# snakers4/silero-vad

Measured on AMD Instinct MI355X. Metric: audio-chunks/sec (32 ms @ 16 kHz), higher is better.
Workload: dtype f32; 1 GPU; configs[1]: synthetic 16 kHz PCM resident in HBM, 512-sample chunks, 4096 streams/GPU x 256 chunks/stream per step, zero initial state; streams_per_gpu=4096

## Files before the change

silero_vad_amd/csrc/device_api.hpp:

```cpp
#pragma once
#include <hip/hip_runtime.h>

#include <cstdint>

#include "../../include/silero_vad_hip.h"

namespace vad {

struct RefNet {
    const float *basis;
    const float *ew[4], *eb[4];
    const float *w_ih, *w_hh, *b_ih, *b_hh, *w_out, *b_out;
};

__device__ __forceinline__ float load_pcm(const float *p) { return *p; }
__device__ __forceinline__ float load_pcm(const int16_t *p) { return (float)(*p) * (1.0f / 32768.0f); }

template <typename PcmT>
hipError_t launch_ref_forward(const RefNet &w, int sr, int B, long L, const PcmT *pcm, long ld,
                              float *ctx, float *state, float *probs, long ldp, hipStream_t s);

template <typename PcmT>
hipError_t launch_decimate(const PcmT *src, long lds, PcmT *dst, long ldd, int B, long Ld, int k, hipStream_t s);

struct FrontArgs {
    const float *wfront;
    const float *tables;
    const void *pcm;
    const void *tail;
    long ld, L, T;
    long t0, nt;
    const float *ctx_in;
    float *ctx_out;
    float *gx;
    int B;
    int dec;
    long long *trace;
    const RefNet *exact_net;
    int *exact_list;
    const float *gx_silent;
};
hipError_t launch_exact_silent(int sr, const RefNet *net_dev, float *out, hipStream_t s);
template <typename PcmT>
hipError_t launch_exact_fix(int sr, const FrontArgs &a, hipStream_t s);
template <typename PcmT>
hipError_t launch_front(int sr, const FrontArgs &a, hipStream_t s);
template <typename PcmT>
hipError_t launch_front_f43(int sr, const FrontArgs &a, hipStream_t s);
template <typename PcmT>
hipError_t launch_front_lat(int sr, const FrontArgs &a, hipStream_t s);
struct CellArgs {
    const float *whh_lat;
    float *state;
    float *probs;
    long ldp;
    const uint8_t *present;
};
template <typename PcmT>
hipError_t launch_step_lat(int sr, const FrontArgs &a, const CellArgs &c, hipStream_t s);
template <typename PcmT>
hipError_t launch_step_one(int sr, const FrontArgs &a, const CellArgs &c, hipStream_t s);
template <typename PcmT>
hipError_t launch_front_one(int sr, const FrontArgs &a, hipStream_t s);
template <typename PcmT>
hipError_t launch_front_wino(int sr, const FrontArgs &a, hipStream_t s);

struct RecArgs {
    const float *whh;
    const float *tables;
    const float *gx;
    float *state;
    float *probs;
    long ldp, t0, nt;
    int B;
    const uint8_t *present;
};
hipError_t launch_rec(int sr, const RecArgs &a, hipStream_t s);
hipError_t launch_carry_absent(const uint8_t *present, const float *ctx_in, float *ctx_out, int C, float *probs, long ldp, int B,
                               hipStream_t s);
hipError_t launch_expand_rows(const uint8_t *present, const int32_t *pos, const uint8_t *src, void *dst, long row_bytes, int B, hipStream_t s);
hipError_t launch_assemble_packets(const int32_t *table, long n_rows, const int16_t *pkt, int16_t *carry, int16_t *batch, int N, hipStream_t s);
constexpr int kCodecShift = 16;
hipError_t launch_assemble_coded_packets(const int32_t *table, long n_rows, const uint8_t *pkt, int16_t *carry, int16_t *batch, int N,
                                         hipStream_t s);
hipError_t launch_assemble_burst(const int32_t *table, long n_rows, const uint8_t *pkt, int16_t *carry, int16_t *batch, int16_t *more,
                                 int max_chunks, int streams, int N, hipStream_t s);
hipError_t launch_burst_flags(const uint8_t *k_of_stream, uint8_t *flags, long ld, int steps, int streams, hipStream_t s);

__host__ __device__ inline int16_t ulaw_to_s16(uint8_t code) {
    const unsigned u = ~code & 0xffu;
    const int t = (int)((((u & 0x0fu) << 3) + 0x84u) << ((u & 0x70u) >> 4));
    return (int16_t)((u & 0x80u) ? 0x84 - t : t - 0x84);
}
__host__ __device__ inline int16_t alaw_to_s16(uint8_t code) {
    const unsigned a = code ^ 0x55u;
    const unsigned seg = (a & 0x70u) >> 4;
    const int m = (int)((a & 0x0fu) << 4);
    const int t = seg == 0 ? m + 8 : (m + 0x108) << (seg - 1);
    return (int16_t)((a & 0x80u) ? t : -t);
}
__host__ __device__ inline int16_t g711_to_s16(int codec, uint8_t code) {
// ... 26 lines not shown
```

silero_vad_amd/csrc/engine.hip:

```cpp
#include <hip/hip_runtime.h>

#include <chrono>

#include <sched.h>

#include <algorithm>
#include <atomic>
#include <cctype>
#include <cstdio>
#include <cstdlib>
#include <cstring>
#include <map>
#include <memory>
#include <mutex>
#include <new>
#include <string>
#include <vector>

#include "../../include/silero_vad_hip.h"
#include "device_api.hpp"
#include "host_threads.hpp"
#include "layout.hpp"
#include "weights.hpp"

#ifndef VAD_AB
#define VAD_AB 0
#endif

struct vad_images {
    int device = -1;
    uint8_t *d_blob = nullptr;
    vad::RefNet ref[2] = {};
    vad::RefNet *d_ref = nullptr;
    float *d_gx_silent = nullptr;
    float *d_front4[2] = {}, *d_whh[2] = {}, *d_whh_lat[2] = {}, *d_whh_rows[2] = {}, *d_tables[2] = {};
    uint16_t *d_whh_b9[2] = {}, *d_front_b9[2] = {};
#if VAD_AB
    float *d_front[2] = {}, *d_front_wino[2] = {};
#endif
    ~vad_images() {
        if (device < 0) return;
        (void)hipSetDevice(device);
        for (int ni = 0; ni < 2; ++ni) {
            if (d_front4[ni]) (void)hipFree(d_front4[ni]);
            if (d_whh[ni]) (void)hipFree(d_whh[ni]);
            if (d_whh_b9[ni]) (void)hipFree(d_whh_b9[ni]);
            if (d_whh_rows[ni]) (void)hipFree(d_whh_rows[ni]);
            if (d_front_b9[ni]) (void)hipFree(d_front_b9[ni]);
            if (d_whh_lat[ni]) (void)hipFree(d_whh_lat[ni]);
            if (d_tables[ni]) (void)hipFree(d_tables[ni]);
#if VAD_AB
            if (d_front[ni]) (void)hipFree(d_front[ni]);
            if (d_front_wino[ni]) (void)hipFree(d_front_wino[ni]);
#endif
        }
        if (d_blob) (void)hipFree(d_blob);
        if (d_ref) (void)hipFree(d_ref);
        if (d_gx_silent) (void)hipFree(d_gx_silent);
    }
};

struct vad_engine {
    std::shared_ptr<vad::Weights> weights;
    std::shared_ptr<vad_images> img;
    bool host_only = false;
    int device = -1;
    std::string err;
    bool impl_reference = false;
    int enc0 = 2;
    bool fuse_step = true;
    int rec_form = 0;
    bool front_b9 = false;
    bool rec_b9 = false;
    bool profile = false;
    bool fused_decimation = true;
    bool exact_all_silent = true;
    bool exact_transitions = true;
    int one_max = 256;
    long lat_tiles = 768;
    long long *trace = nullptr;

    float *d_gx = nullptr;
    size_t gx_floats = 0;
    float *d_ctx_new = nullptr;
    size_t ctx_floats = 0;
    int *d_exact = nullptr;
    size_t exact_ints = 0;
    void *d_tail = nullptr;
    size_t tail_bytes = 0;
    void *d_realign = nullptr;
    size_t realign_bytes = 0;
    void *d_decim = nullptr;
    size_t decim_bytes = 0;
    unsigned long scratch_gen = 0;
    long slab_steps = 0;
    size_t gx_cap = 6ull << 30;

    static constexpr int kTabSlots = 8;
    vad::RowDesc *h_tab[kTabSlots] = {};
    long tab_cap[kTabSlots] = {};
    hipEvent_t tab_ev[kTabSlots] = {};
    bool tab_busy[kTabSlots] = {};
    int tab_next = 0;

    static constexpr int kDmaStreams = 4;
    hipStream_t dma_stream[kDmaStreams] = {};
    hipEvent_t dma_fork = nullptr, dma_join[kDmaStreams] = {};

    const void *map_host[2] = {nullptr, nullptr};
    void *map_dev[2] = {nullptr, nullptr};
    unsigned long map_gen = 0;

    std::vector<hipEvent_t> ev_pool;
    size_t ev_used = 0;
    long prof_calls = 0;
};

namespace {

int fail(vad_engine *e, int code, const std::string &msg) {
    if (e) e->err = msg;
    return code;
}
// ... 147 lines not shown
        ra.tables = e->img->d_tables[ni];
        ra.gx = e->d_gx;
        ra.state = state;
        ra.probs = probs;
        ra.ldp = ldp; ra.t0 = t0; ra.nt = nt; ra.B = B;
        ra.present = present;
        hipEvent_t *ev = nullptr;
        if (prof) {
            while (e->ev_pool.size() < e->ev_used + 3) {
                hipEvent_t x;
                HIP_TRY(e, hipEventCreate(&x));
                e->ev_pool.push_back(x);
            }
            ev = &e->ev_pool[e->ev_used];
            e->ev_used += 3;
            HIP_TRY(e, hipEventRecord(ev[0], stream));
        }
        const long tiles = (long)((B + 15) / 16) * nt;
        const bool one = T == 1 && dec == 1 && B <= e->one_max && !e->rec_b9 && !e->front_b9 && e->enc0 == 2;
        if (T == 1 && e->fuse_step && !e->rec_b9 && !e->front_b9 && e->enc0 == 2 && (tiles <= e->lat_tiles || one)) {
            vad::CellArgs ca{};
            ca.whh_lat = e->img->d_whh_lat[ni];
            ca.state = state;
            ca.probs = probs;
            ca.ldp = ldp;
            ca.present = present;
            if (one) {
                if (!ctx_next) {
                    fa.ctx_out = ctx;
                    ctx_in_place = true;
                }
                HIP_TRY(e, vad::launch_step_one<PcmT>(sr, fa, ca, stream));
            } else HIP_TRY(e, vad::launch_step_lat<PcmT>(sr, fa, ca, stream));
            if (prof) {
                HIP_TRY(e, hipEventRecord(ev[1], stream));
                HIP_TRY(e, hipEventRecord(ev[2], stream));
            }
            continue;
        }
        bool front_stamped = false;
        if (e->front_b9) {
            fa.wfront = reinterpret_cast<const float *>(e->img->d_front_b9[ni]);
            HIP_TRY(e, vad::launch_front_b9<PcmT>(sr, fa, stream));
        } else
#if VAD_AB
        if (e->enc0 == 1) HIP_TRY(e, vad::launch_front_wino<PcmT>(sr, fa, stream));
        else if (e->enc0 == 0) HIP_TRY(e, vad::launch_front<PcmT>(sr, fa, stream));
        else
#endif
        if (one) HIP_TRY(e, vad::launch_front_one<PcmT>(sr, fa, stream));
        else if (tiles <= e->lat_tiles) HIP_TRY(e, vad::launch_front_lat<PcmT>(sr, fa, stream));
        else {
            fa.exact_list = exact ? e->d_exact : nullptr;
            HIP_TRY(e, vad::launch_front_f43<PcmT>(sr, fa, stream));
            if (prof) HIP_TRY(e, hipEventRecord(ev[1], stream));
            front_stamped = prof;
            HIP_TRY(e, vad::launch_exact_fix<PcmT>(sr, fa, stream));
        }
        if (prof && !front_stamped) HIP_TRY(e, hipEventRecord(ev[1], stream));
        if (e->rec_b9) HIP_TRY(e, vad::launch_rec_b9(sr, ra, stream));
        else if (e->rec_form != 1 && B <= vad::kRecSmallMaxB) {
            ra.whh = e->img->d_whh_rows[ni];
            HIP_TRY(e, vad::launch_rec_small(sr, ra, stream));
        } else HIP_TRY(e, vad::launch_rec(sr, ra, stream));
        if (prof) HIP_TRY(e, hipEventRecord(ev[2], stream));
    }
    if (present) HIP_TRY(e, vad::launch_carry_absent(present, ctx, ctx_next ? ctx_next : ctx_in_place ? nullptr : e->d_ctx_new, C, probs, ldp, B, stream));
    if (!ctx_next && !ctx_in_place) HIP_TRY(e, hipMemcpyAsync(ctx, e->d_ctx_new, (size_t)B * C * sizeof(float), hipMemcpyDeviceToDevice, stream));
    return VAD_OK;
}

template <typename PcmT>
int forward_impl(vad_engine *e, int sr, int B, long L, const PcmT *pcm, long ld, float *ctx,
                 float *state, float *probs, long ldp, void *stream_v) {
    if (!e) return VAD_ERR_ARG;
    if (e->host_only) return fail(e, VAD_ERR_NO_DEVICE, "host-only engine");
    if (B < 0 || L < 0 || (B > 0 && L > 0 && (!pcm || !ctx || !state || !probs)) || ld < L)
        return fail(e, VAD_ERR_ARG, "bad argument");
    hipStream_t stream = (hipStream_t)stream_v;
    if (sr > 16000 && sr % 16000 == 0) {
        if (B == 0 || L == 0) return VAD_OK;
        const int k = sr / 16000;
        HIP_TRY(e, hipSetDevice(e->device));
        if ((k == 2 || (k == 3 && e->enc0 == 2)) && !e->impl_reference && e->fused_decimation)
            return forward_core<PcmT>(e, 16000, k, B, L, pcm, ld, ctx, state, probs, ldp, stream);
        const long Ld = (L + k - 1) / k, ldd = (Ld + 15) / 16 * 16;
        int rc = grow(e, &e->d_decim, &e->decim_bytes, (size_t)B * ldd * sizeof(PcmT), stream, "decimation");
        if (rc) return rc;
        PcmT *dec = reinterpret_cast<PcmT *>(e->d_decim);
        HIP_TRY(e, vad::launch_decimate<PcmT>(pcm, ld, dec, ldd, B, Ld, k, stream));
        return forward_impl<PcmT>(e, 16000, B, Ld, dec, ldd, ctx, state, probs, ldp, stream_v);
    }
    const int ni = net_index(sr);
    if (ni < 0) return fail(e, VAD_ERR_SAMPLE_RATE, "Supported sampling rates: [8000, 16000] (or multiply of 16000)");
    if (B == 0 || L == 0) return VAD_OK;
    HIP_TRY(e, hipSetDevice(e->device));
    if (e->impl_reference) {
        const int N = sr == 16000 ? 512 : 256;
        if (ldp < (L + N - 1) / N) return fail(e, VAD_ERR_ARG, "ldp < T");
        HIP_TRY(e, vad::launch_ref_forward<PcmT>(e->img->ref[ni], sr, B, L, pcm, ld, ctx, state, probs, ldp, stream));
        return VAD_OK;
    }
    return forward_core<PcmT>(e, sr, 1, B, L, pcm, ld, ctx, state, probs, ldp, stream);
}

template <typename T>
int upload(vad_engine *e, T **dst, const std::vector<T> &src) {
// ... 11 lines not shown
        case VAD_OK: return "ok";
        case VAD_ERR_ARG: return "invalid argument";
        case VAD_ERR_SAMPLE_RATE: return "unsupported sampling rate (supported: 8000, 16000)";
        case VAD_ERR_WEIGHTS: return "malformed weight container";
        case VAD_ERR_NO_DEVICE: return "no usable gfx950 HIP device";
        case VAD_ERR_HIP: return "HIP runtime error";
        case VAD_ERR_ALLOC: return "device allocation failed";
        case VAD_ERR_CAPTURE: return "scratch growth during stream capture";
        case VAD_ERR_OPTION: return "unknown option";
        default: return "unknown status";
    }
}

const char *vad_last_error(const vad_engine *e) { return e ? e->err.c_str() : "null engine"; }
int vad_device(const vad_engine *e) { return e ? e->device : -1; }

int vad_geometry(int sr, int *chunk, int *context) {
    if (net_index(sr) < 0) return VAD_ERR_SAMPLE_RATE;
    if (chunk) *chunk = sr == 16000 ? 512 : 256;
    if (context) *context = sr == 16000 ? 64 : 32;
    return VAD_OK;
}

int vad_create_host_only(const void *weights, size_t nbytes, vad_engine **out) {
    if (!out) return VAD_ERR_ARG;
    *out = nullptr;
    vad_engine *e = new (std::nothrow) vad_engine();
    if (!e) return VAD_ERR_ALLOC;
    e->weights = std::make_shared<vad::Weights>();
    const std::string err = e->weights->load(weights, nbytes);
    if (!err.empty()) {
        delete e;
        return VAD_ERR_WEIGHTS;
    }
    e->host_only = true;
    *out = e;
    return VAD_OK;
}

int vad_create(const void *weights, size_t nbytes, int device, vad_engine **out) {
    if (!out) return VAD_ERR_ARG;
    *out = nullptr;
    int ndev = 0;
    if (hipGetDeviceCount(&ndev) != hipSuccess || ndev <= 0 || device < 0 || device >= ndev)
        return VAD_ERR_NO_DEVICE;
    hipDeviceProp_t prop;
    if (hipGetDeviceProperties(&prop, device) != hipSuccess) return VAD_ERR_NO_DEVICE;
    if (std::strncmp(prop.gcnArchName, "gfx950", 6) != 0) return VAD_ERR_NO_DEVICE;
    vad_engine *e = nullptr;
    int rc = vad_create_host_only(weights, nbytes, &e);
    if (rc) return rc;
    e->host_only = false;
    e->device = device;
    auto bail = [&](int code) {
        vad_destroy(e);
        return code;
    };
    if (hipSetDevice(device) != hipSuccess) return bail(VAD_ERR_HIP);
    e->img = std::make_shared<vad_images>();
    vad_images &im = *e->img;
    im.device = device;
    for (int ni = 0; ni < 2; ++ni) {
        const vad::PackedNet &pk = e->weights->packed[ni];
        if (upload(e, &im.d_front4[ni], pk.front_wino4)) return bail(VAD_ERR_HIP);
        if (upload(e, &im.d_whh[ni], pk.whh)) return bail(VAD_ERR_HIP);
        if (upload(e, &im.d_whh_b9[ni], pk.whh_b9)) return bail(VAD_ERR_HIP);
        if (upload(e, &im.d_front_b9[ni], pk.front_b9)) return bail(VAD_ERR_HIP);
        if (upload(e, &im.d_whh_lat[ni], pk.whh_lat)) return bail(VAD_ERR_HIP);
        if (upload(e, &im.d_whh_rows[ni], pk.whh_rows)) return bail(VAD_ERR_HIP);
        if (upload(e, &im.d_tables[ni], pk.tables)) return bail(VAD_ERR_HIP);
#if VAD_AB
        if (upload(e, &im.d_front[ni], pk.front)) return bail(VAD_ERR_HIP);
        if (upload(e, &im.d_front_wino[ni], pk.front_wino)) return bail(VAD_ERR_HIP);
#endif
    }
    const auto &blob = e->weights->blob;
    if (hipMalloc((void **)&im.d_blob, blob.size()) != hipSuccess) return bail(VAD_ERR_ALLOC);
    if (hipMemcpy(im.d_blob, blob.data(), blob.size(), hipMemcpyHostToDevice) != hipSuccess)
        return bail(VAD_ERR_HIP);
    for (int ni = 0; ni < 2; ++ni) {
        const vad::NetTensors &t = e->weights->net[ni];
        auto dev = [&](const float *p) {
            return reinterpret_cast<const float *>(im.d_blob + ((const uint8_t *)p - blob.data()));
        };
        vad::RefNet &r = im.ref[ni];
        r.basis = dev(t.basis);
        for (int l = 0; l < 4; ++l) { r.ew[l] = dev(t.ew[l]); r.eb[l] = dev(t.eb[l]); }
        r.w_ih = dev(t.w_ih); r.w_hh = dev(t.w_hh); r.b_ih = dev(t.b_ih); r.b_hh = dev(t.b_hh);
        r.w_out = dev(t.w_out); r.b_out = dev(t.b_out);
    }
    if (hipMalloc((void **)&im.d_ref, sizeof(im.ref)) != hipSuccess) return bail(VAD_ERR_ALLOC);
    if (hipMemcpy(im.d_ref, im.ref, sizeof(im.ref), hipMemcpyHostToDevice) != hipSuccess) return bail(VAD_ERR_HIP);
    if (hipMalloc((void **)&im.d_gx_silent, 2 * 512 * sizeof(float)) != hipSuccess) return bail(VAD_ERR_ALLOC);
    for (int ni = 0; ni < 2; ++ni)
        if (vad::launch_exact_silent(ni == 0 ? 16000 : 8000, im.d_ref + ni, im.d_gx_silent + 512 * ni, nullptr) != hipSuccess) return bail(VAD_ERR_HIP);
    if (hipDeviceSynchronize() != hipSuccess) return bail(VAD_ERR_HIP);
    *out = e;
    return VAD_OK;
}

void vad_destroy(vad_engine *e) {
    if (e && e->dma_fork) {
        (void)hipSetDevice(e->device);
        for (int k = 0; k < vad_engine::kDmaStreams; ++k) {
            if (e->dma_stream[k]) { (void)hipStreamSynchronize(e->dma_stream[k]); (void)hipStreamDestroy(e->dma_stream[k]); }
            if (e->dma_join[k]) (void)hipEventDestroy(e->dma_join[k]);
        }
        (void)hipEventDestroy(e->dma_fork);
        e->dma_fork = nullptr;
    }
    if (!e) return;
    if (!e->host_only && e->device >= 0) {
        (void)hipSetDevice(e->device);
        (void)hipDeviceSynchronize();
        if (e->d_gx) (void)hipFree(e->d_gx);
        if (e->d_ctx_new) (void)hipFree(e->d_ctx_new);
        if (e->d_exact) (void)hipFree(e->d_exact);
        if (e->d_tail) (void)hipFree(e->d_tail);
        if (e->d_realign) (void)hipFree(e->d_realign);
        if (e->d_decim) (void)hipFree(e->d_decim);
        for (int i = 0; i < vad_engine::kTabSlots; ++i) {
            if (e->h_tab[i]) (void)hipHostFree(e->h_tab[i]);
            if (e->tab_ev[i]) (void)hipEventDestroy(e->tab_ev[i]);
        }
        for (auto &ev : e->ev_pool) (void)hipEventDestroy(ev);
    }
    delete e;
}

int vad_clone(const vad_engine *src, vad_engine **out) {
    if (!src || !out) return VAD_ERR_ARG;
    *out = nullptr;
    if (src->host_only) return VAD_ERR_NO_DEVICE;
    vad_engine *e = new (std::nothrow) vad_engine();
    if (!e) return VAD_ERR_ALLOC;
    e->weights = src->weights;
    e->img = src->img;
    e->device = src->device;
    e->impl_reference = src->impl_reference;
    e->enc0 = src->enc0;
    e->fused_decimation = src->fused_decimation;
    e->lat_tiles = src->lat_tiles;
    e->rec_b9 = src->rec_b9;
    e->rec_form = src->rec_form;
    e->front_b9 = src->front_b9;
    e->fuse_step = src->fuse_step;
    e->one_max = src->one_max;
    e->exact_transitions = src->exact_transitions;
    e->exact_all_silent = src->exact_all_silent;
    e->gx_cap = src->gx_cap;
    e->trace = src->trace;
    *out = e;
    return VAD_OK;
}

int vad_set_option(vad_engine *e, const char *name, const char *value) {
    if (!e || !name || !value) return VAD_ERR_ARG;
    const std::string n(name), v(value);
    if (n == "impl") {
        if (v == "mfma") e->impl_reference = false;
        else if (v == "reference") e->impl_reference = true;
        else return fail(e, VAD_ERR_OPTION, "impl must be mfma|reference");
        return VAD_OK;
    }
    if (n == "precision") {
        if (v != "fp32") return fail(e, VAD_ERR_OPTION, "precision must be fp32 (the engine computes in fp32 only)");
        return VAD_OK;
    }
    if (n == "enc0") {
        if (v == "winograd" || v == "winograd4") e->enc0 = 2;
#if VAD_AB
        else if (v == "winograd2") e->enc0 = 1;
        else if (v == "direct") e->enc0 = 0;
        else return fail(e, VAD_ERR_OPTION, "enc0 must be winograd|winograd4|winograd2|direct");
#else
        else return fail(e, VAD_ERR_OPTION, "enc0 must be winograd (the A/B forms winograd2|direct exist only in the test build, "
                                            "libsilero_vad_hip_ab.so)");
#endif
        return VAD_OK;
    }
    if (n == "rec") {
        if (v == "fp32") e->rec_b9 = false;
        else if (v == "bf16x9") e->rec_b9 = true;
        else return fail(e, VAD_ERR_OPTION, "rec must be fp32|bf16x9");
        return VAD_OK;
    }
    if (n == "front_mma") {
        if (v == "fp32") e->front_b9 = false;
        else if (v == "bf16x9") e->front_b9 = true;
        else return fail(e, VAD_ERR_OPTION, "front_mma must be fp32|bf16x9");
        return VAD_OK;
    }
    if (n == "rec_form") {
        if (v == "auto" || v == "valu") e->rec_form = 0;
        else if (v == "mfma") e->rec_form = 1;
        else return fail(e, VAD_ERR_OPTION, "rec_form must be auto|mfma|valu");
        return VAD_OK;
    }
    if (n == "fuse_step") {
        e->fuse_step = (v != "0");
        return VAD_OK;
    }
    if (n == "front") {
        if (v == "auto") e->lat_tiles = 768;
        else if (v == "throughput") e->lat_tiles = 0;
        else if (v == "latency") e->lat_tiles = 0x7fffffffL;
        else return fail(e, VAD_ERR_OPTION, "front must be auto|throughput|latency");
        return VAD_OK;
    }
    if (n == "step_one") {
        if (v == "auto") e->one_max = 256;
        else {
            char *end = nullptr;
            const long k = std::strtol(v.c_str(), &end, 10);
            if (!end || *end || k < 0 || k > 4096) return fail(e, VAD_ERR_OPTION, "step_one: auto | 0 .. 4096");
            e->one_max = (int)k;
        }
        return VAD_OK;
    }
    if (n == "exact_transitions") {
        if (v != "0" && v != "1" && v != "edges") return fail(e, VAD_ERR_OPTION, "exact_transitions: 0 | 1 (| edges: study mode)");
        e->exact_transitions = v != "0";
        e->exact_all_silent = v == "1";
        return VAD_OK;
    }
    if (n == "fused_decimation") {
        e->fused_decimation = (v != "0");
        return VAD_OK;
    }
    if (n == "gx_cap_mib") {
        const long mib = std::strtol(value, nullptr, 0);
        if (mib < 1) return fail(e, VAD_ERR_OPTION, "gx_cap_mib must be >= 1");
        e->gx_cap = (size_t)mib << 20;
        return VAD_OK;
    }
    if (n == "trace_ptr") {
        e->trace = reinterpret_cast<long long *>(std::strtoull(value, nullptr, 0));
        return VAD_OK;
    }
    if (n == "profile") {
        e->profile = (v == "1");
        e->ev_used = 0;
        e->prof_calls = 0;
        return VAD_OK;
    }
    return fail(e, VAD_ERR_OPTION, "unknown option " + n);
}

int vad_step(vad_engine *e, int sr, int B, const float *pcm, long ld, float *ctx, float *state,
             float *prob, void *stream) {
    const int N = (sr > 16000 && sr % 16000 == 0) ? 512 * (sr / 16000) : sr == 16000 ? 512 : 256;
    return forward_impl<float>(e, sr, B, N, pcm, ld, ctx, state, prob, 1, stream);
}
// ... 263 lines not shown
    if (!e || kind < 0 || kind > 1 || blocks < 0 || iters < 0) return VAD_ERR_ARG;
    if (e->host_only) return fail(e, VAD_ERR_NO_DEVICE, "host-only engine");
    HIP_TRY(e, hipSetDevice(e->device));
    HIP_TRY(e, vad::launch_foreign_spin(e->img->d_tables[0], blocks, iters, kind, (hipStream_t)stream));
    return VAD_OK;
}

int vad_debug_frontend(vad_engine *e, int sr, int B, long L, const float *pcm, long ld,
                       const float *ctx, float *gx, void *stream_v) {
    if (!e) return VAD_ERR_ARG;
    if (e->host_only) return fail(e, VAD_ERR_NO_DEVICE, "host-only engine");
    const int ni = net_index(sr);
    if (ni < 0) return fail(e, VAD_ERR_SAMPLE_RATE, "bad sr");
    if (B <= 0 || L <= 0 || !pcm || !ctx || !gx) return fail(e, VAD_ERR_ARG, "bad argument");
    const int N = sr == 16000 ? 512 : 256;
    const long T = (L + N - 1) / N;
    hipStream_t stream = (hipStream_t)stream_v;
    HIP_TRY(e, hipSetDevice(e->device));
    int rc = ensure_scratch(e, sr, B, T, stream);
    if (rc) return rc;
    if (e->slab_steps < T) return fail(e, VAD_ERR_ARG, "debug frontend: input too long");
    if (L % N || ((size_t)pcm & 15) || (ld * sizeof(float)) % 16 || ((size_t)ctx & 15))
        return fail(e, VAD_ERR_ARG, "debug frontend: whole chunks and 16-byte aligned rows only");
    vad::FrontArgs fa{};
#if VAD_AB
    fa.wfront = e->enc0 == 2 ? e->img->d_front4[ni] : e->enc0 == 1 ? e->img->d_front_wino[ni] : e->img->d_front[ni];
#else
    fa.wfront = e->img->d_front4[ni];
#endif
    fa.tables = e->img->d_tables[ni];
    fa.pcm = pcm;
    fa.ld = ld; fa.L = L; fa.T = T; fa.t0 = 0; fa.nt = T;
    fa.ctx_in = ctx;
    fa.ctx_out = nullptr;
    fa.gx = e->d_gx;
    fa.B = B;
    fa.trace = e->trace;
    const bool exact = e->exact_transitions && e->enc0 == 2 && !e->front_b9;
    fa.exact_net = exact ? e->img->d_ref + ni : nullptr;
    fa.gx_silent = exact && e->exact_all_silent ? e->img->d_gx_silent + 512 * ni : nullptr;
    if (e->front_b9) {
        fa.wfront = reinterpret_cast<const float *>(e->img->d_front_b9[ni]);
        HIP_TRY(e, vad::launch_front_b9<float>(sr, fa, stream));
    } else
#if VAD_AB
    if (e->enc0 == 1) HIP_TRY(e, vad::launch_front_wino<float>(sr, fa, stream));
    else if (e->enc0 == 0) HIP_TRY(e, vad::launch_front<float>(sr, fa, stream));
    else
#endif
    if (T == 1 && B <= e->one_max && e->enc0 == 2) HIP_TRY(e, vad::launch_front_one<float>(sr, fa, stream));
    else if ((long)((B + 15) / 16) * T <= e->lat_tiles) HIP_TRY(e, vad::launch_front_lat<float>(sr, fa, stream));
    else {
        fa.exact_list = exact ? e->d_exact : nullptr;
        HIP_TRY(e, vad::launch_front_f43<float>(sr, fa, stream));
        HIP_TRY(e, vad::launch_exact_fix<float>(sr, fa, stream));
    }
    HIP_TRY(e, vad::launch_unpack_gx(e->d_gx, gx, B, T, stream));
    return VAD_OK;
}


namespace {
struct Registered {
    size_t bytes;
    void *dev;
};
std::mutex g_reg_mutex;
std::map<const uint8_t *, Registered> g_registered;

const void *device_view(const void *p) {
    {
        std::lock_guard<std::mutex> g(g_reg_mutex);
        if (!g_registered.empty()) {
            auto it = g_registered.upper_bound(static_cast<const uint8_t *>(p));
            if (it != g_registered.begin()) {
                --it;
                const size_t off = static_cast<const uint8_t *>(p) - it->first;
                if (off < it->second.bytes) return static_cast<const uint8_t *>(it->second.dev) + off;
            }
        }
    }
    void *dev = nullptr;
    if (hipHostGetDevicePointer(&dev, const_cast<void *>(p), 0) != hipSuccess || !dev) {
        (void)hipGetLastError();
        return nullptr;
    }
    return dev;
}
}

int vad_host_register(void *p, size_t bytes) {
    if (!p || !bytes) return VAD_ERR_ARG;
    if (hipHostRegister(p, bytes, hipHostRegisterMapped | hipHostRegisterPortable) != hipSuccess) {
        (void)hipGetLastError();
        return VAD_ERR_HIP;
    }
    void *dev = nullptr;
    if (hipHostGetDevicePointer(&dev, p, 0) != hipSuccess || !dev) dev = p;
    std::lock_guard<std::mutex> g(g_reg_mutex);
    g_registered[static_cast<const uint8_t *>(p)] = Registered{bytes, dev};
    return VAD_OK;
}

int vad_host_unregister(void *p) {
    if (!p) return VAD_ERR_ARG;
    {
        std::lock_guard<std::mutex> g(g_reg_mutex);
// ... 169 lines not shown
```

silero_vad_amd/csrc/kernel_front_f43.hip:

```cpp
#include <hip/hip_runtime.h>

#include <type_traits>

#include "fft_wave.hpp"
#include "exact_front.hpp"
#include "front_common.hpp"

namespace vad {
namespace {

#ifndef VAD_BV_BATCH
#define VAD_BV_BATCH 1
#endif
constexpr int kUnitBytes = (int)vadl::kWUnitFloats * 4;
struct Ring {
    unsigned a_cur, a_nxt, a_far;
    unsigned d_cur, d_nxt, d_far;
    const float *src;
    unsigned voff;
    f32x4 c0, c1;
};

__device__ __forceinline__ void ring_request(Ring &r) {
    if (VAD_ABLATE & 8) return;
    unsigned keep_m0;
    asm volatile("s_mov_b32 %0, m0\n\ts_mov_b32 m0, %3\n\ts_nop 0\n\t"
                 "global_load_lds_dwordx4 %1, %2\n\tglobal_load_lds_dwordx4 %1, %2 offset:1024\n\t"
                 "global_load_lds_dwordx4 %1, %2 offset:2048\n\tglobal_load_lds_dwordx4 %1, %2 offset:3072\n\t"
                 "s_mov_b32 m0, %0"
                 : "=&s"(keep_m0) : "v"(r.voff), "s"(r.src), "s"(r.d_far) : "memory");
    r.src += vadl::kWUnitFloats;
}
__device__ __forceinline__ void ring_rotate(Ring &r) {
    const unsigned a = r.a_cur, d = r.d_cur;
    r.a_cur = r.a_nxt; r.a_nxt = r.a_far; r.a_far = a;
    r.d_cur = r.d_nxt; r.d_nxt = r.d_far; r.d_far = d;
}

template <int M, int KG, int AFTER, class BF>
__device__ __forceinline__ void gemm_r(f32x4 (&acc)[M], BF bfun, Ring &r) {
    constexpr int NSTEPS = KG * (M / 2), NU = NSTEPS / 8;
    static_assert(NSTEPS % 8 == 0 && M % 2 == 0, "segments are whole units");
    static_for<0, NU>([&](auto uc) VAD_INLINE {
        constexpr int u = decltype(uc)::value, after = (NU - 1 - u) + AFTER;
        static_for<0, 8>([&](auto sc_) VAD_INLINE {
            constexpr int st = decltype(sc_)::value;
            if constexpr (st == 4 && after >= 1) {
                asm volatile("s_waitcnt vmcnt(0)" ::: "memory");
                if (!(VAD_ABLATE & 1)) __builtin_amdgcn_s_barrier();
                asm volatile("" ::: "memory");
                if constexpr (after >= 2) ring_request(r);
            }
            f32x4 n0 = r.c0, n1 = r.c1;
            if constexpr (st + 1 < 8) {
                n0 = lds4(r.a_cur + (2 * (st + 1)) * 1024);
                n1 = lds4(r.a_cur + (2 * (st + 1) + 1) * 1024);
            } else if constexpr (after >= 1) {
                n0 = lds4(r.a_nxt);
                n1 = lds4(r.a_nxt + 1024);
            }
            __builtin_amdgcn_sched_barrier(0);
            constexpr int i = u * 8 + st, kg = i / (M / 2), mp = 2 * (i % (M / 2));
#if VAD_BV_BATCH
            float bv[4];
#pragma unroll
            for (int ks = 0; ks < 4; ++ks) bv[ks] = bfun(kg * 4 + ks);
            __builtin_amdgcn_sched_barrier(0);
#pragma unroll
            for (int ks = 0; ks < 4; ++ks) {
                acc[mp + 0] = __builtin_amdgcn_mfma_f32_16x16x4f32(r.c0[ks], bv[ks], acc[mp + 0], 0, 0, 0);
                acc[mp + 1] = __builtin_amdgcn_mfma_f32_16x16x4f32(r.c1[ks], bv[ks], acc[mp + 1], 0, 0, 0);
            }
#else
#pragma unroll
            for (int ks = 0; ks < 4; ++ks) {
                const float bv = bfun(kg * 4 + ks);
                acc[mp + 0] = __builtin_amdgcn_mfma_f32_16x16x4f32(r.c0[ks], bv, acc[mp + 0], 0, 0, 0);
                acc[mp + 1] = __builtin_amdgcn_mfma_f32_16x16x4f32(r.c1[ks], bv, acc[mp + 1], 0, 0, 0);
            }
#endif
            __builtin_amdgcn_sched_barrier(0);
            r.c0 = n0;
            r.c1 = n1;
        });
        ring_rotate(r);
    });
}

#ifndef VAD_F43_GEMM_PRIO
#define VAD_F43_GEMM_PRIO 0
#endif
#ifndef VAD_F43_FFT_PRIO
#define VAD_F43_FFT_PRIO 0
#endif
template <int Q, typename PcmT, int DEC>
__global__ void __launch_bounds__(256, 2) front_f43_kernel(const FrontArgs a) {
    using namespace vadl;
    constexpr Tab tb = make_tab(8 * Q, Q);
    constexpr int TABF = (tb.total + 3) / 4 * 4;
    constexpr int RB = w_rb(Q), P = w_parts(Q), KG0 = Q / 4;
    constexpr int PB = Q == 32 ? 2 : 1;
    static_assert(w4_tail0(Q) + 20 == w4_units(Q) && P % PB == 0, "program mismatch");
    __shared__ __attribute__((aligned(16))) float lds[TABF + 3 * (kUnitBytes / 4)];
    float *tab = lds;

    Lane ln;
    ln.lane = threadIdx.x & 63;
    ln.wave = __builtin_amdgcn_readfirstlane(threadIdx.x >> 6);
    ln.g = ln.lane >> 4;
    ln.j = ln.lane & 15;
    const long nst = (a.B + 15) / 16, total = nst * a.nt;
    long wt = (long)blockIdx.x * 4 + ln.wave;
    ln.tile_valid = wt < total;
    if (!ln.tile_valid) wt = total - 1;
    ln.tl = wt % a.nt;
    ln.st = wt / a.nt;
    ln.t = a.t0 + ln.tl;
    const long bb = ln.st * 16 + ln.j;
    ln.b = (int)(bb < a.B ? bb : a.B - 1);
    ln.from_tail = a.tail != nullptr && ln.t == a.T - 1;
    ln.sgnA = ln.g < 2 ? 1.f : -1.f;
    ln.sgnB = (ln.g & 1) ? -1.f : 1.f;
#if VAD_TRACE
    VAD_WAVE_STAMP(ln, 0);
#endif

    Ring ring;
    {
        const unsigned slot0 = (unsigned)(size_t)((__attribute__((address_space(3))) float *)(lds + TABF));
        ring.voff = ln.lane * 16;
        ring.a_cur = slot0 + ring.voff;
        ring.a_nxt = ring.a_cur + kUnitBytes;
        ring.a_far = ring.a_cur + 2 * kUnitBytes;
        ring.d_far = slot0 + (unsigned)ln.wave * 4096u;
        ring.d_cur = ring.d_far + kUnitBytes;
        ring.d_nxt = ring.d_far + 2 * kUnitBytes;
        ring.src = a.wfront + ln.wave * 1024;
        ring_request(ring);
        {   const unsigned d = ring.d_far; ring.d_far = ring.d_cur; ring.d_cur = ring.d_nxt; ring.d_nxt = d; }
        ring_request(ring);
        {   const unsigned d = ring.d_far; ring.d_far = ring.d_cur; ring.d_cur = ring.d_nxt; ring.d_nxt = d; }
    }
    {
        static_assert(tb.total % 4 == 0, "tables are copied as 16-byte vectors");
        constexpr int NV = tb.total / 4, PER = (NV + 255) / 256;
        const f32x4 *src = reinterpret_cast<const f32x4 *>(a.tables);
        f32x4 v[PER];
#pragma unroll
        for (int k = 0; k < PER; ++k) {
            const int i = threadIdx.x + k * 256;
            v[k] = src[i < NV ? i : NV - 1];
        }
#pragma unroll
        for (int k = 0; k < PER; ++k) {
            const int i = threadIdx.x + k * 256;
            if (i < NV) reinterpret_cast<f32x4 *>(tab)[i] = v[k];
        }
    }
    asm volatile("s_waitcnt vmcnt(0)" ::: "memory");
    __syncthreads();
    VAD_WAVE_STAMP(ln, 1);

    float X0[Q + 1], X1[Q + 1], X2[Q + 1], X3[Q + 1];
#pragma unroll
    for (int k = 0; k <= Q; ++k) X1[k] = X2[k] = X3[k] = 0.f;
#pragma clang loop unroll(disable)
    for (int v = 0; v < 4; ++v) {
        if (v >= 3) {
#pragma unroll
            for (int k = 0; k <= Q; ++k) X0[k] = X1[k];
        }
        if (v >= 2) {
#pragma unroll
            for (int k = 0; k <= Q; ++k) X1[k] = X2[k];
        }
        if (v >= 1) {
#pragma unroll
            for (int k = 0; k <= Q; ++k) X2[k] = X3[k];
        }
        if (VAD_F43_FFT_PRIO) __builtin_amdgcn_s_setprio(VAD_F43_FFT_PRIO);
        fft_frame<Q, PcmT, DEC>(X3, v, a, tab, ln);
        if (VAD_F43_FFT_PRIO) __builtin_amdgcn_s_setprio(0);
    }
    if (VAD_F43_GEMM_PRIO) __builtin_amdgcn_s_setprio(VAD_F43_GEMM_PRIO);
    const float xn0 = __shfl(X0[Q], ln.j), xn1 = __shfl(X1[Q], ln.j), xn2 = __shfl(X2[Q], ln.j), xn3 = __shfl(X3[Q], ln.j);
    if (!VAD_NO_EXACT && a.exact_list != nullptr) {
        const SilentMasks sm = silent_chunks(X0[0], X1[0], X2[0], X3[0]);
        const long left = (long)a.B - ln.st * 16;
        const unsigned take = (sm.edge | (a.gx_silent != nullptr ? sm.silent : 0u)) & (left >= 16 ? 0xffffu : ((1u << left) - 1u));
        if (take != 0 && ln.tile_valid) {
            int base = 0;
            if (ln.lane == 0) base = atomicAdd(a.exact_list, __builtin_popcount(take));
            base = __shfl(base, 0);
            if (ln.g == 0 && ((take >> ln.j) & 1))
                a.exact_list[2 + base + __builtin_popcount(take & ((1u << ln.j) - 1u))] =
                    (int)(wt * 16 + ln.j) | (((sm.silent >> ln.j) & 1) ? kExactSilentBit : 0);
        }
    }

#if VAD_F43_EF
#pragma unroll
    for (int k = 0; k < Q; ++k) {
        X3[k] = X3[k] - X1[k];
        X0[k] = X2[k] - X0[k];
    }
    float poison;
    {   float p0 = 0.f, p1 = 0.f;
        poison_acc<Q>(p0, p1, X3);
        poison_acc<Q>(p0, p1, X0);
        poison = poison_nyq(p0, p1, xn0, xn1, xn2, xn3);
    }
#else
    float poison;
    {   float p0 = 0.f, p1 = 0.f;
// ... 109 lines not shown
                gemm_r<4, 4, 2>(Z1, [&](int s) VAD_INLINE { return one(Y2, s); }, ring);
                gemm_r<4, 4, 2>(Z1, [&](int s) VAD_INLINE { return one(Y3, s); }, ring);
            }
        });
    }
    add_bias<4>(Z0, tab + tb.b_e1, ln);
    add_bias<4>(Z1, tab + tb.b_e1, ln);
    relu<4>(Z0);
    relu<4>(Z1);
    VAD_WAVE_STAMP(ln, 10);

    f32x4 Vv[4];
    auto bZ0 = [&](int s) VAD_INLINE { return Z0[s >> 2][s & 3]; };
    auto bZ1 = [&](int s) VAD_INLINE { return Z1[s >> 2][s & 3]; };
    auto bV = [&](int s) VAD_INLINE { return Vv[s >> 2][s & 3]; };
    init_bias<4>(Vv, tab + tb.b_e2, ln);
    gemm_r<4, 4, 2>(Vv, bZ0, ring);
    gemm_r<4, 4, 2>(Vv, bZ1, ring);
    relu<4>(Vv);
    f32x4 Fe[8];
    auto bF = [&](int s) VAD_INLINE { return Fe[s >> 2][s & 3]; };
    init_bias<8>(Fe, tab + tb.b_e3, ln);
    gemm_r<8, 4, 2>(Fe, bV, ring);
    relu<8>(Fe);
    poison_into(Fe[0], poison);
    VAD_WAVE_STAMP(ln, 11);

    float *gxt = a.gx + ((size_t)(ln.st * a.nt + ln.tl) * 32) * 256 + ln.lane * 4;
    const float *bg = tab + tb.b_g;
#pragma clang loop unroll(disable)
    for (int q = 0; q < 3; ++q) {
        f32x4 G[8];
        init_bias<8>(G, bg, ln);
        gemm_r<8, 8, 2>(G, bF, ring);
        if (ln.tile_valid) {
#pragma unroll
            for (int m = 0; m < 8; ++m) *reinterpret_cast<f32x4 *>(gxt + (size_t)m * 256) = G[m];
        }
        gxt += 8 * 256;
        bg += 128;
    }
    {
        f32x4 G[8];
        init_bias<8>(G, bg, ln);
        gemm_r<8, 8, 0>(G, bF, ring);
        if (ln.tile_valid) {
#pragma unroll
            for (int m = 0; m < 8; ++m) *reinterpret_cast<f32x4 *>(gxt + (size_t)m * 256) = G[m];
        }
    }
#if VAD_TRACE
    VAD_WAVE_STAMP(ln, 12);
    if (a.trace && ln.lane == 0) {
        long long *tr = a.trace + ((size_t)blockIdx.x * 4 + ln.wave) * 32;
#pragma unroll
        for (int k = 0; k < 20; ++k) tr[k] = (long long)ln.ts[k];
        tr[13] = __builtin_amdgcn_s_getreg((31 << 11) | 4);
        tr[14] = __builtin_amdgcn_s_getreg((31 << 11) | 20);
        tr[15] = (long long)wall_clock64();
    }
#endif
}

}

template <typename PcmT>
hipError_t launch_front_f43(int sr, const FrontArgs &a, hipStream_t s) {
    if (a.B <= 0 || a.nt <= 0) return hipSuccess;
    const long nst = (a.B + 15) / 16, total = nst * a.nt;
    const unsigned grid = (unsigned)((total + 3) / 4);
    if (a.dec > 1 && (sr != 16000 || a.dec > 3)) return hipErrorInvalidValue;
    if (a.dec == 3) hipLaunchKernelGGL((front_f43_kernel<32, PcmT, 3>), dim3(grid), dim3(256), 0, s, a);
    else if (a.dec == 2) hipLaunchKernelGGL((front_f43_kernel<32, PcmT, 2>), dim3(grid), dim3(256), 0, s, a);
    else if (sr == 16000) hipLaunchKernelGGL((front_f43_kernel<32, PcmT, 1>), dim3(grid), dim3(256), 0, s, a);
    else hipLaunchKernelGGL((front_f43_kernel<16, PcmT, 1>), dim3(grid), dim3(256), 0, s, a);
    return hipGetLastError();
}
template hipError_t launch_front_f43<float>(int, const FrontArgs &, hipStream_t);
template hipError_t launch_front_f43<int16_t>(int, const FrontArgs &, hipStream_t);

}
```

Baseline: 190.3 million chunks/s.

## Add persistent front kernel that loops tiles and prefetches weights across tiles

Adds a persistent variant of the f43 front-end kernel launched with 2 workgroups per CU, where each workgroup loops over tile groups. The table copy and weight ring prologue run once per workgroup, and the weight ring restarts at the tail of one tile so the next tile's first units are already in flight. This removes per-block prologue and launch costs and the pipeline bubble between tiles. The cost is more complex ring phase bookkeeping and possible load imbalance from the fixed grid size. It is enabled by default.

Measured after the change: 186.3 million chunks/s. 2.1% lower.

```diff
diff --git a/silero_vad_amd/csrc/device_api.hpp b/silero_vad_amd/csrc/device_api.hpp
--- a/silero_vad_amd/csrc/device_api.hpp
+++ b/silero_vad_amd/csrc/device_api.hpp
@@ -46,7 +46,7 @@
 template <typename PcmT>
 hipError_t launch_front(int sr, const FrontArgs &a, hipStream_t s);
 template <typename PcmT>
-hipError_t launch_front_f43(int sr, const FrontArgs &a, hipStream_t s);
+hipError_t launch_front_f43(int sr, const FrontArgs &a, hipStream_t s, int persist_wgs);
 template <typename PcmT>
 hipError_t launch_front_lat(int sr, const FrontArgs &a, hipStream_t s);
 struct CellArgs {
diff --git a/silero_vad_amd/csrc/engine.hip b/silero_vad_amd/csrc/engine.hip
--- a/silero_vad_amd/csrc/engine.hip
+++ b/silero_vad_amd/csrc/engine.hip
@@ -69,6 +69,8 @@
     bool impl_reference = false;
     int enc0 = 2;
     bool fuse_step = true;
+    bool front_persist = true;
+    int front_wgs = 0;
     int rec_form = 0;
     bool front_b9 = false;
     bool rec_b9 = false;
@@ -322,7 +324,7 @@
         else if (tiles <= e->lat_tiles) HIP_TRY(e, vad::launch_front_lat<PcmT>(sr, fa, stream));
         else {
             fa.exact_list = exact ? e->d_exact : nullptr;
-            HIP_TRY(e, vad::launch_front_f43<PcmT>(sr, fa, stream));
+            HIP_TRY(e, vad::launch_front_f43<PcmT>(sr, fa, stream, e->front_persist ? e->front_wgs : 0));
             if (prof) HIP_TRY(e, hipEventRecord(ev[1], stream));
             front_stamped = prof;
             HIP_TRY(e, vad::launch_exact_fix<PcmT>(sr, fa, stream));
@@ -440,6 +442,7 @@
     if (rc) return rc;
     e->host_only = false;
     e->device = device;
+    e->front_wgs = 2 * prop.multiProcessorCount;
     auto bail = [&](int code) {
         vad_destroy(e);
         return code;
@@ -533,6 +536,8 @@
     e->rec_form = src->rec_form;
     e->front_b9 = src->front_b9;
     e->fuse_step = src->fuse_step;
+    e->front_persist = src->front_persist;
+    e->front_wgs = src->front_wgs;
     e->one_max = src->one_max;
     e->exact_transitions = src->exact_transitions;
     e->exact_all_silent = src->exact_all_silent;
@@ -587,6 +592,12 @@
     }
     if (n == "fuse_step") {
         e->fuse_step = (v != "0");
+        return VAD_OK;
+    }
+    if (n == "front_persist") {
+        if (v == "1") e->front_persist = true;
+        else if (v == "0") e->front_persist = false;
+        else return fail(e, VAD_ERR_OPTION, "front_persist must be 1|0");
         return VAD_OK;
     }
     if (n == "front") {
@@ -956,7 +967,7 @@
     else if ((long)((B + 15) / 16) * T <= e->lat_tiles) HIP_TRY(e, vad::launch_front_lat<float>(sr, fa, stream));
     else {
         fa.exact_list = exact ? e->d_exact : nullptr;
-        HIP_TRY(e, vad::launch_front_f43<float>(sr, fa, stream));
+        HIP_TRY(e, vad::launch_front_f43<float>(sr, fa, stream, e->front_persist ? e->front_wgs : 0));
         HIP_TRY(e, vad::launch_exact_fix<float>(sr, fa, stream));
     }
     HIP_TRY(e, vad::launch_unpack_gx(e->d_gx, gx, B, T, stream));
diff --git a/silero_vad_amd/csrc/kernel_front_f43.hip b/silero_vad_amd/csrc/kernel_front_f43.hip
--- a/silero_vad_amd/csrc/kernel_front_f43.hip
+++ b/silero_vad_amd/csrc/kernel_front_f43.hip
@@ -19,6 +19,8 @@
     const float *src;
     unsigned voff;
     f32x4 c0, c1;
+    const float *src0;
+    bool more;
 };
 
 __device__ __forceinline__ void ring_request(Ring &r) {
@@ -50,6 +52,17 @@
                 if (!(VAD_ABLATE & 1)) __builtin_amdgcn_s_barrier();
                 asm volatile("" ::: "memory");
                 if constexpr (after >= 2) ring_request(r);
+                else if (r.more) {
+                    r.src = r.src0;
+                    ring_request(r);
+                }
+            } else if constexpr (st == 4) {
+                if (r.more) {
+                    asm volatile("s_waitcnt vmcnt(0)" ::: "memory");
+                    if (!(VAD_ABLATE & 1)) __builtin_amdgcn_s_barrier();
+                    asm volatile("" ::: "memory");
+                    ring_request(r);
+                }
             }
             f32x4 n0 = r.c0, n1 = r.c1;
             if constexpr (st + 1 < 8) {
@@ -93,24 +106,66 @@
 #ifndef VAD_F43_FFT_PRIO
 #define VAD_F43_FFT_PRIO 0
 #endif
-template <int Q, typename PcmT, int DEC>
-__global__ void __launch_bounds__(256, 2) front_f43_kernel(const FrontArgs a) {
+template <int Q>
+struct FrontLds {
+    static constexpr vadl::Tab tb = vadl::make_tab(8 * Q, Q);
+    static constexpr int TABF = (tb.total + 3) / 4 * 4;
+    static constexpr int FLOATS = TABF + 3 * (kUnitBytes / 4);
+};
+
+template <int Q>
+__device__ __forceinline__ void front_prologue(const FrontArgs &a, float *lds, unsigned slot0) {
+    constexpr vadl::Tab tb = FrontLds<Q>::tb;
+    const int lane = threadIdx.x & 63, wave = __builtin_amdgcn_readfirstlane(threadIdx.x >> 6);
+    {
+        Ring ring;
+        ring.voff = lane * 16;
+        ring.src = a.wfront + wave * 1024;
+        ring.d_far = slot0 + (unsigned)wave * 4096u;
+        ring_request(ring);
+        ring.d_far += kUnitBytes;
+        ring_request(ring);
+    }
+    {
+        static_assert(tb.total % 4 == 0, "tables are copied as 16-byte vectors");
+        constexpr int NV = tb.total / 4, PER = (NV + 255) / 256;
+        const f32x4 *src = reinterpret_cast<const f32x4 *>(a.tables);
+        f32x4 v[PER];
+#pragma unroll
+        for (int k = 0; k < PER; ++k) {
+            const int i = threadIdx.x + k * 256;
+            v[k] = src[i < NV ? i : NV - 1];
+        }
+#pragma unroll
+        for (int k = 0; k < PER; ++k) {
+            const int i = threadIdx.x + k * 256;
+            if (i < NV) reinterpret_cast<f32x4 *>(lds)[i] = v[k];
+        }
+    }
+    asm volatile("s_waitcnt vmcnt(0)" ::: "memory");
+    __syncthreads();
+}
+
+template <int Q, typename PcmT, int DEC, bool LOOPED>
+__device__ __forceinline__ void front_f43_tile(const long grp, const FrontArgs &a, float *tab, const unsigned slot0,
+                                               const unsigned phase, const bool more, const unsigned long long seam) {
     using namespace vadl;
-    constexpr Tab tb = make_tab(8 * Q, Q);
-    constexpr int TABF = (tb.total + 3) / 4 * 4;
+    constexpr Tab tb = FrontLds<Q>::tb;
     constexpr int RB = w_rb(Q), P = w_parts(Q), KG0 = Q / 4;
     constexpr int PB = Q == 32 ? 2 : 1;
     static_assert(w4_tail0(Q) + 20 == w4_units(Q) && P % PB == 0, "program mismatch");
-    __shared__ __attribute__((aligned(16))) float lds[TABF + 3 * (kUnitBytes / 4)];
-    float *tab = lds;
 
     Lane ln;
-    ln.lane = threadIdx.x & 63;
+    if constexpr (LOOPED) {
+        asm volatile("v_mbcnt_lo_u32_b32 %0, -1, 0\n\tv_mbcnt_hi_u32_b32 %0, -1, %0" : "=v"(ln.lane));
+    } else {
+        ln.lane = threadIdx.x & 63;
+    }
     ln.wave = __builtin_amdgcn_readfirstlane(threadIdx.x >> 6);
     ln.g = ln.lane >> 4;
     ln.j = ln.lane & 15;
     const long nst = (a.B + 15) / 16, total = nst * a.nt;
-    long wt = (long)blockIdx.x * 4 + ln.wave;
+    long wt = grp * 4 + ln.wave;
     ln.tile_valid = wt < total;
     if (!ln.tile_valid) wt = total - 1;
     ln.tl = wt % a.nt;
@@ -127,39 +182,20 @@
 
     Ring ring;
     {
-        const unsigned slot0 = (unsigned)(size_t)((__attribute__((address_space(3))) float *)(lds + TABF));
+        const unsigned s_cur = phase * kUnitBytes, s_nxt = (phase == 2 ? 0 : phase + 1) * kUnitBytes,
+                       s_far = (phase == 0 ? 2 : phase - 1) * kUnitBytes;
         ring.voff = ln.lane * 16;
-        ring.a_cur = slot0 + ring.voff;
-        ring.a_nxt = ring.a_cur + kUnitBytes;
-        ring.a_far = ring.a_cur + 2 * kUnitBytes;
-        ring.d_far = slot0 + (unsigned)ln.wave * 4096u;
-        ring.d_cur = ring.d_far + kUnitBytes;
-        ring.d_nxt = ring.d_far + 2 * kUnitBytes;
-        ring.src = a.wfront + ln.wave * 1024;
-        ring_request(ring);
-        {   const unsigned d = ring.d_far; ring.d_far = ring.d_cur; ring.d_cur = ring.d_nxt; ring.d_nxt = d; }
-        ring_request(ring);
-        {   const unsigned d = ring.d_far; ring.d_far = ring.d_cur; ring.d_cur = ring.d_nxt; ring.d_nxt = d; }
-    }
-    {
-        static_assert(tb.total % 4 == 0, "tables are copied as 16-byte vectors");
-        constexpr int NV = tb.total / 4, PER = (NV + 255) / 256;
-        const f32x4 *src = reinterpret_cast<const f32x4 *>(a.tables);
-        f32x4 v[PER];
-#pragma unroll
-        for (int k = 0; k < PER; ++k) {
-            const int i = threadIdx.x + k * 256;
-            v[k] = src[i < NV ? i : NV - 1];
-        }
-#pragma unroll
-        for (int k = 0; k < PER; ++k) {
-            const int i = threadIdx.x + k * 256;
-            if (i < NV) reinterpret_cast<f32x4 *>(tab)[i] = v[k];
-        }
-    }
-    asm volatile("s_waitcnt vmcnt(0)" ::: "memory");
-    __syncthreads();
-    VAD_WAVE_STAMP(ln, 1);
+        ring.a_cur = slot0 + s_cur + ring.voff;
+        ring.a_nxt = slot0 + s_nxt + ring.voff;
+        ring.a_far = slot0 + s_far + ring.voff;
+        const unsigned d0 = slot0 + (unsigned)ln.wave * 4096u;
+        ring.d_cur = d0 + s_cur;
+        ring.d_nxt = d0 + s_nxt;
+        ring.d_far = d0 + s_far;
+        ring.src0 = a.wfront + ln.wave * 1024;
+        ring.src = ring.src0 + 2 * kWUnitFloats;
+        ring.more = more;
+    }
 
     float X0[Q + 1], X1[Q + 1], X2[Q + 1], X3[Q + 1];
 #pragma unroll
@@ -375,31 +411,67 @@
 #if VAD_TRACE
     VAD_WAVE_STAMP(ln, 12);
     if (a.trace && ln.lane == 0) {
-        long long *tr = a.trace + ((size_t)blockIdx.x * 4 + ln.wave) * 32;
+        long long *tr = a.trace + ((size_t)grp * 4 + ln.wave) * 32;
 #pragma unroll
         for (int k = 0; k < 20; ++k) tr[k] = (long long)ln.ts[k];
         tr[13] = __builtin_amdgcn_s_getreg((31 << 11) | 4);
         tr[14] = __builtin_amdgcn_s_getreg((31 << 11) | 20);
         tr[15] = (long long)wall_clock64();
-    }
-#endif
+        tr[20] = (long long)seam;
+        tr[21] = (long long)blockIdx.x;
+    }
+#endif
+}
+
+template <int Q, typename PcmT, int DEC>
+__global__ void __launch_bounds__(256, 2) front_f43_kernel(const FrontArgs a) {
+    __shared__ __attribute__((aligned(16))) float lds[FrontLds<Q>::FLOATS];
+    const unsigned slot0 = (unsigned)(size_t)((__attribute__((address_space(3))) float *)(lds + FrontLds<Q>::TABF));
+    front_prologue<Q>(a, lds, slot0);
+    front_f43_tile<Q, PcmT, DEC, false>((long)blockIdx.x, a, lds, slot0, 0u, false, 0ull);
+}
+
+template <int Q, typename PcmT, int DEC>
+__global__ void __launch_bounds__(256, 2) front_f43_persist_kernel(const FrontArgs a) {
+    __shared__ __attribute__((aligned(16))) float lds[FrontLds<Q>::FLOATS];
+    const unsigned lds_base = (unsigned)(size_t)((__attribute__((address_space(3))) float *)lds);
+    front_prologue<Q>(a, lds, lds_base + FrontLds<Q>::TABF * 4);
+    const long nst = (a.B + 15) / 16, total = nst * a.nt;
+    const unsigned ngrp = (unsigned)((total + 3) / 4), G = gridDim.x;
+    unsigned phase = 0;
+    unsigned long long seam = 0;
+    for (unsigned grp = blockIdx.x; grp < ngrp; grp += G) {
+        const bool more = grp + G < ngrp;
+        front_f43_tile<Q, PcmT, DEC, true>((long)grp, a, lds, lds_base + FrontLds<Q>::TABF * 4, phase, more, seam);
+#if VAD_TRACE
+        seam = __builtin_readcyclecounter();
+#endif
+        phase = (phase + vadl::w4_units(Q)) % 3;
+    }
 }
 
 }
 
 template <typename PcmT>
-hipError_t launch_front_f43(int sr, const FrontArgs &a, hipStream_t s) {
+hipError_t launch_front_f43(int sr, const FrontArgs &a, hipStream_t s, int persist_wgs) {
     if (a.B <= 0 || a.nt <= 0) return hipSuccess;
     const long nst = (a.B + 15) / 16, total = nst * a.nt;
-    const unsigned grid = (unsigned)((total + 3) / 4);
+    const unsigned groups = (unsigned)((total + 3) / 4);
+    const unsigned grid = persist_wgs > 0 ? (groups < (unsigned)persist_wgs ? groups : (unsigned)persist_wgs) : groups;
     if (a.dec > 1 && (sr != 16000 || a.dec > 3)) return hipErrorInvalidValue;
-    if (a.dec == 3) hipLaunchKernelGGL((front_f43_kernel<32, PcmT, 3>), dim3(grid), dim3(256), 0, s, a);
-    else if (a.dec == 2) hipLaunchKernelGGL((front_f43_kernel<32, PcmT, 2>), dim3(grid), dim3(256), 0, s, a);
-    else if (sr == 16000) hipLaunchKernelGGL((front_f43_kernel<32, PcmT, 1>), dim3(grid), dim3(256), 0, s, a);
-    else hipLaunchKernelGGL((front_f43_kernel<16, PcmT, 1>), dim3(grid), dim3(256), 0, s, a);
+#define VAD_F43_LAUNCH(K)                                                                                      \
+    do {                                                                                                       \
+        if (a.dec == 3) hipLaunchKernelGGL((K<32, PcmT, 3>), dim3(grid), dim3(256), 0, s, a);                   \
+        else if (a.dec == 2) hipLaunchKernelGGL((K<32, PcmT, 2>), dim3(grid), dim3(256), 0, s, a);              \
+        else if (sr == 16000) hipLaunchKernelGGL((K<32, PcmT, 1>), dim3(grid), dim3(256), 0, s, a);             \
+        else hipLaunchKernelGGL((K<16, PcmT, 1>), dim3(grid), dim3(256), 0, s, a);                              \
+    } while (0)
+    if (persist_wgs > 0) VAD_F43_LAUNCH(front_f43_persist_kernel);
+    else VAD_F43_LAUNCH(front_f43_kernel);
+#undef VAD_F43_LAUNCH
     return hipGetLastError();
 }
-template hipError_t launch_front_f43<float>(int, const FrontArgs &, hipStream_t);
-template hipError_t launch_front_f43<int16_t>(int, const FrontArgs &, hipStream_t);
-
-}
+template hipError_t launch_front_f43<float>(int, const FrontArgs &, hipStream_t, int);
+template hipError_t launch_front_f43<int16_t>(int, const FrontArgs &, hipStream_t, int);
+
+}
```
